# TritonDataCenter/containerpilot

Hardware: NVIDIA H100
Metric: events/sec through Bus.Publish (deliveries/s = 32-byte records landed in subscriber mailboxes) (higher is better)
Workload: dtype u8

## Files before the change

containerpilot_b200/csrc/cpbus.cu:

```cuda
#include "cpbus_kernels.cuh"

#include <algorithm>
#include <chrono>
#include <cstdio>
#include <cstdlib>
#include <cstring>
#include <deque>
#include <mutex>
#include <new>
#include <string>
#include <thread>
#include <unordered_map>
#include <vector>

using namespace cpbus_dev;

namespace {

thread_local char g_cuda_err[256] = "";

#define CK(call)                                                                                   \
  do {                                                                                             \
    cudaError_t e_ = (call);                                                                       \
    if (e_ != cudaSuccess) {                                                                       \
// ... 74 lines not shown
  unsigned long long* d_follow_clock = nullptr;
  int follow_next = 0;
  cudaEvent_t follow_done = nullptr;
  std::recursive_mutex follow_mu;
  DevPubAcct* d_acct = nullptr;
  DevPubAcct* h_acct = nullptr;
  std::deque<DbgItem> dbg_pending;
  PairCounter pub_pairs;
  cpbus_event* d_drain = nullptr; size_t drain_cap = 0;
  uint2* d_drain_idx = nullptr; size_t drain_idx_cap = 0;
  unsigned long long* d_ready_lb = nullptr; size_t ready_lb_tiles = 0;
  cpbus_ready* d_ready = nullptr; uint32_t* d_ready_slot = nullptr; size_t ready_stage_cap = 0;
  unsigned long long* h_ready_hdr = nullptr;
  unsigned long long* d_ready_hdr = nullptr;
  uint32_t subs_per_warp = 0;
  uint32_t order_block = 0;
  bool pdl = true;
  cudaEvent_t launched = nullptr;
  int hints = -1;
  static constexpr int kFoldSlots = 8;
  unsigned long long* d_fold = nullptr;
  cudaEvent_t fold_done[kFoldSlots] = {};
  uint32_t fold_next = 0;
  static constexpr int kStage = 8;
  static constexpr int kDevSlots = 64, kDevEpoch = 16;
  cpbus_event* d_stage = nullptr;
  cudaEvent_t epoch_done[kDevSlots / kDevEpoch] = {};
  uint32_t dev_slot = 0;
  cpbus_event* h_batch[kStage] = {};
  cudaEvent_t h2d_done[kStage] = {};
  cudaStream_t copy_stream = nullptr;
  cudaStream_t result_stream = nullptr;
  DevResultSlot* d_result = nullptr;
  DevResultSlot* h_result = nullptr;
  cudaEvent_t result_done[8] = {};
  uint32_t result_next = 0;
  DevStats* h_stats = nullptr;
  unsigned long long* h_fold = nullptr;
  int cur = 0;
  size_t n_staged = 0;

  std::vector<uint32_t> h_mask;
  std::vector<uint8_t> h_active;
  std::vector<uint8_t> h_npairs;
  uint2* d_pairs = nullptr;
  uint32_t n_paired = 0;
  uint32_t* d_order = nullptr;
  uint32_t n_order = 0, n_filtered = 0;
  bool order_dirty = true;
  std::vector<size_t> oneshot_idx;
  std::vector<HostTimer> h_timers;
  uint32_t n_next = 0, n_active = 0, n_timers = 0;
  uint64_t min_period = UINT64_MAX;

  uint64_t now = 0, last_watermark = 0, seq = 0;
  uint64_t room_lb = 0;

  int dbg_head = -1, dbg_tail = 0;
  cpbus_event dbg[10]{};

  std::unordered_map<std::string, uint32_t> intern;
  std::vector<std::string> sources;
  size_t intern_bytes = 0;
  struct EphSlot { std::string s; uint32_t gen = 0; bool live = false; };
  std::vector<EphSlot> eph;
  std::unordered_map<std::string, uint32_t> eph_map;
  uint32_t eph_next = 0;
  uint64_t eph_live = 0, eph_recycled = 0;
  std::vector<cpbus_stream*> streams;

  cpbus_stats_t st{};
  std::mutex mu;
};

namespace {

int rebuild_order(cpbus* b);

int dev_guard(cpbus* b) {
  CK(cudaSetDevice(b->device));
  return CPBUS_OK;
}

int stream_error(const cpbus* b) {
  const unsigned int e = *(volatile const unsigned int*)b->h_err;
  return (e & kErrFollowOrder) ? CPBUS_EORDER : (e ? CPBUS_ETIMEDOUT : CPBUS_OK);
}

uint32_t mask_word(const cpbus* b, uint32_t local) {
  uint32_t hint = 0;
  if (b->K && !b->h_timers.empty())
    for (uint32_t k = 0; k < b->K; k++)
// ... 38 lines not shown
    const size_t base = order.size();
    order.resize(base + count.back());
    for (uint32_t i = lo; i < hi; i++) if (!active || active[i]) order[base + count[masks[i] & CPBUS_MASK_ALL]++] = i;
    if (heavy_first) {
      const size_t nb = order.size() - base;
      uint32_t pc_count[34] = {};
      for (size_t k = 0; k < nb; k++) pc_count[32 - __builtin_popcount(masks[order[base + k]] & CPBUS_MASK_ALL) + 1]++;
      for (int k = 1; k < 34; k++) pc_count[k] += pc_count[k - 1];
      tmp.resize(nb);
      for (size_t k = 0; k < nb; k++) tmp[pc_count[32 - __builtin_popcount(masks[order[base + k]] & CPBUS_MASK_ALL)]++] = order[base + k];
      std::copy(tmp.begin(), tmp.end(), order.begin() + base);
    }
  }
}

int rebuild_order(cpbus* b) {
  std::vector<uint32_t> order;
  static_assert(sizeof(b->h_active[0]) == 1, "h_active is a byte vector");
  mask_order(b->h_mask.data(), reinterpret_cast<const uint8_t*>(b->h_active.data()), b->n_next, b->R, b->order_block, true, order);
  b->n_order = (uint32_t)order.size();
  if (b->n_order) {
    CK(cudaMemcpyAsync(b->d_order, order.data(), (size_t)b->n_order * 4, cudaMemcpyHostToDevice, b->stream));
    CK(cudaStreamSynchronize(b->stream));
  }
  b->order_dirty = false;
  return CPBUS_OK;
}

constexpr int kFanoutMaxSmem = 200 * 1024;

template <int STORE, bool TIMERS, bool DIGEST, bool ORDERED, bool PAIRS = false>
int launch_fanout_t(cpbus* b, const FanoutParams& p, uint32_t grid, size_t smem, bool follow) {
  static bool attr_done[2][64] = {};
  void (*kernel)(FanoutParams) = follow ? fanout_follow_kernel<STORE, TIMERS, DIGEST, ORDERED, PAIRS>
                                        : fanout_kernel<STORE, TIMERS, DIGEST, ORDERED, PAIRS>;
  const int dev = b->device & 63;
  if (!attr_done[follow][dev]) {
    CK(cudaFuncSetAttribute(kernel, cudaFuncAttributeMaxDynamicSharedMemorySize, kFanoutMaxSmem));
    attr_done[follow][dev] = true;
  }
  cudaLaunchConfig_t cfg{};
  cfg.gridDim = dim3(grid); cfg.blockDim = dim3(kThreads); cfg.dynamicSmemBytes = smem; cfg.stream = b->stream;
  cudaLaunchAttribute attr[1];
  attr[0].id = cudaLaunchAttributeProgrammaticStreamSerialization;
  attr[0].val.programmaticStreamSerializationAllowed = 1;
  cfg.attrs = attr; cfg.numAttrs = b->pdl ? 1 : 0;
  CK(cudaLaunchKernelEx(&cfg, kernel, p));
  CK(cudaGetLastError());
  return CPBUS_OK;
}
// ... 32 lines not shown
    p.follow_from_host = sa->follow_from_host ? 1u : 0u;
  }
  p.prefetch_src = prefetch_src; p.prefetch_dst = prefetch_dst; p.prefetch_n = prefetch_n;
  p.batch_dep = batch_dep ? 1u : 0u; p.n_ev = n;
  p.n_subs = b->n_next; p.ring_cap = b->R; p.K = b->K; p.sub_base = b->cfg.sub_id_base;
  p.use_digest = b->use_digest; p.lossless = b->lossless; p.timers_on = b->n_timers > 0 && b->K > 0;
  p.smem_cap = (n + 31u) & ~31u;
  const size_t hot_bytes = (size_t)b->n_next * (sizeof(SubCtl) + (p.timers_on ? b->K * sizeof(DevTimer) : 0));
  p.hints = b->hints >= 0 ? (uint32_t)b->hints : (hot_bytes <= (64u << 20) ? 1u : 0u);
  const uint32_t need = (b->n_next + kWarpsPerCta - 1) / kWarpsPerCta;
  uint32_t grid = b->cfg.grid_ctas ? std::max(1u, std::min(b->cfg.grid_ctas, need)) : 0u;
  int rc;
  const bool pairs_on = b->n_paired > 0 && b->d_pairs;
  p.pairs = pairs_on ? b->d_pairs : nullptr;
  size_t smem = fanout_smem_bytes(p.smem_cap) + (pairs_on ? kPairFilterBytes : 0);
  if (!pairs_on && !p.timers_on && b->n_filtered > 0) {
    if (b->order_dirty) { const int rc_order = rebuild_order(b); if (rc_order) return rc_order; }
    if (b->n_order) {
      const uint32_t scale = std::max(1u, (p.n_ev + 128u) / 256u);
      uint32_t spw = b->subs_per_warp ? std::min(32u, b->subs_per_warp)
                                      : std::max(4u, std::min(16u / scale, b->n_order / (20480u * scale)));
      p.order = b->d_order; p.n_order = b->n_order; p.spw = spw;
      const uint32_t warps = (b->n_order + spw - 1) / spw;
      grid = std::max(1u, (warps + kWarpsPerCta - 1) / kWarpsPerCta);
    }
  }
  if (pairs_on && !b->cfg.grid_ctas) {
    const uint32_t blocks = (b->n_next + 31u) / 32u;
    grid = std::max(1u, std::min((blocks + kWarpsPerCta - 1) / kWarpsPerCta, (uint32_t)b->sm_count * 16u));
  }
  if (!pairs_on && !p.order) {
    uint32_t spw = b->subs_per_warp;
    if (grid) spw = std::max(1u, (need + grid - 1) / grid);
    else if (!spw) {
      const uint32_t scale = std::max(1u, (p.n_ev + 128u) / 256u);
      const uint32_t cap = std::max(1u, 16u / scale);
      spw = std::max(1u, std::min(cap, (need + (uint32_t)b->sm_count * 7 * scale) / ((uint32_t)b->sm_count * 14 * scale)));
    }
    p.spw = spw;
    grid = std::max(1u, (need + spw - 1) / spw);
    const size_t off = fanout_stage_off(p.smem_cap);
    const size_t per_sub = sizeof(SubCtl) + (p.timers_on ? (size_t)b->K * sizeof(DevTimer) : 0);
    const size_t min_round = (size_t)kWarpsPerCta * per_sub;
    const size_t ctas = std::max<size_t>(1, std::min<size_t>(kCtasPerSm, b->smem_per_sm / (off + min_round + b->smem_reserved)));
    const size_t room = std::min<size_t>(kFanoutMaxSmem, b->smem_per_sm / ctas - b->smem_reserved) - off;
    p.stage_subs = std::max<uint32_t>(kWarpsPerCta, (uint32_t)std::min<size_t>((size_t)kWarpsPerCta * spw, room / per_sub) & ~7u);
    smem = off + p.stage_subs * per_sub;
  }
  const int variant = pairs_on ? (p.use_digest ? 7 : 6) : (p.timers_on ? 2 : 0) | (p.use_digest ? 1 : 0) | (p.order ? 4 : 0);
#define CPBUS_DISPATCH(ST)                                                                \
  switch (variant) {                                                                     \
    case 0: rc = launch_fanout_t<ST, false, false, false>(b, p, grid, smem, follow); break;      \
    case 1: rc = launch_fanout_t<ST, false, true, false>(b, p, grid, smem, follow); break;       \
    case 2: rc = launch_fanout_t<ST, true, false, false>(b, p, grid, smem, follow); break;       \
    case 3: rc = launch_fanout_t<ST, true, true, false>(b, p, grid, smem, follow); break;        \
    case 4: rc = launch_fanout_t<ST, false, false, true>(b, p, grid, smem, follow); break;       \
    case 5: rc = launch_fanout_t<ST, false, true, true>(b, p, grid, smem, follow); break;        \
    case 6: rc = launch_fanout_t<ST, true, false, false, true>(b, p, grid, smem, follow); break; \
    default: rc = launch_fanout_t<ST, true, true, false, true>(b, p, grid, smem, follow); break; \
  }
  switch (b->store) {
    case CPBUS_STORE_V4: CPBUS_DISPATCH(CPBUS_STORE_V4); break;
    case CPBUS_STORE_BULK: CPBUS_DISPATCH(CPBUS_STORE_BULK); break;
    default: CPBUS_DISPATCH(CPBUS_STORE_V8); break;
// ... 206 lines not shown
  int ndev = 0;
  if (cudaGetDeviceCount(&ndev) != cudaSuccess || ndev == 0) {
    snprintf(g_cuda_err, sizeof(g_cuda_err), "no CUDA device visible");
    return CPBUS_ENODEV;
  }
  cpbus* b = new (std::nothrow) cpbus();
  if (!b) return CPBUS_ENOMEM;
  b->cfg = *cfg; b->cfg.ring_cap = R; b->cfg.batch_cap = B;
  b->N = cfg->n_max_subs; b->R = R; b->B = B; b->K = K;
  b->lossless = cfg->flags & CPBUS_CFG_LOSSLESS; b->use_digest = cfg->flags & CPBUS_CFG_DIGEST;
  b->room_lb = R;
  b->store = cfg->store_path == CPBUS_STORE_AUTO ? CPBUS_STORE_V8 : (int)cfg->store_path;
  if (const char* e = getenv("CPBUS_PDL")) b->pdl = atoi(e) != 0;
  if (const char* e = getenv("CPBUS_HINTS")) b->hints = atoi(e);
  if (const char* e = getenv("CPBUS_SUBS_PER_WARP")) b->subs_per_warp = (uint32_t)atoi(e);
  if (const char* e = getenv("CPBUS_ORDER_BLOCK")) b->order_block = (uint32_t)atoll(e);
  int rc = CPBUS_OK;
  auto fail = [&](int code) { cpbus_destroy(b); return code; };
  if (cfg->device >= 0) b->device = cfg->device;
  else if (cudaGetDevice(&b->device) != cudaSuccess) return fail(CPBUS_ECUDA);
  if (b->device >= ndev) return fail(CPBUS_EINVAL);
  if ((rc = dev_guard(b))) return fail(rc);
  cudaDeviceProp prop{};
  if (cudaGetDeviceProperties(&prop, b->device) == cudaSuccess) {
    b->sm_count = prop.multiProcessorCount;
    b->smem_per_sm = prop.sharedMemPerMultiprocessor; b->smem_reserved = prop.reservedSharedMemPerBlock;
  }
  if (cfg->stream) b->stream = (cudaStream_t)cfg->stream;
  else {
    if (cudaStreamCreateWithFlags(&b->stream, cudaStreamNonBlocking) != cudaSuccess) return fail(CPBUS_ECUDA);
    b->own_stream = true;
  }
  const size_t N = b->N;
#define ALLOC(ptr, bytes)                                                                     \
  if (cudaMalloc((void**)&(ptr), (bytes)) != cudaSuccess) {                                   \
    snprintf(g_cuda_err, sizeof(g_cuda_err), "cudaMalloc(%zu) failed", (size_t)(bytes));     \
    return fail(CPBUS_ENOMEM);                                                                \
  }
  ALLOC(b->d_ring, N * R * sizeof(cpbus_event));
  ALLOC(b->d_ctl, N * sizeof(SubCtl)); ALLOC(b->d_order, N * 4);
  if (K) ALLOC(b->d_timers, N * K * sizeof(DevTimer));
  ALLOC(b->d_stats, sizeof(DevStats)); ALLOC(b->d_fold, 32 * cpbus::kFoldSlots); ALLOC(b->d_pow, kPowTableLen * 8);
  ALLOC(b->d_desc, 2 * ((fanout_desc_bytes(2048) + 255) & ~(size_t)255)); ALLOC(b->d_desc_ready, 256);
  if (cudaMemsetAsync(b->d_desc_ready, 0, 256, b->stream) != cudaSuccess) return fail(CPBUS_ECUDA);
  if (cudaStreamCreateWithFlags(&b->copy_stream, cudaStreamNonBlocking) != cudaSuccess) return fail(CPBUS_ECUDA);
  if (cudaStreamCreateWithFlags(&b->result_stream, cudaStreamNonBlocking) != cudaSuccess) return fail(CPBUS_ECUDA);
  if (cudaEventCreateWithFlags(&b->launched, cudaEventDisableTiming) != cudaSuccess) return fail(CPBUS_ECUDA);
  ALLOC(b->d_stage, (size_t)cpbus::kDevSlots * B * sizeof(cpbus_event));
  for (int i = 0; i < cpbus::kDevSlots / cpbus::kDevEpoch; i++)
    if (cudaEventCreateWithFlags(&b->epoch_done[i], cudaEventDisableTiming) != cudaSuccess) return fail(CPBUS_ECUDA);
  for (int i = 0; i < cpbus::kStage; i++) {
    if (cudaMallocHost((void**)&b->h_batch[i], (size_t)B * sizeof(cpbus_event)) != cudaSuccess) return fail(CPBUS_ENOMEM);
    if (cudaEventCreateWithFlags(&b->h2d_done[i], cudaEventDisableTiming) != cudaSuccess) return fail(CPBUS_ECUDA);
  }
  ALLOC(b->d_batch_local, (size_t)B * sizeof(cpbus_event));
// ... 34 lines not shown
  b->intern.emplace(std::string(), 0u);
  b->sources.emplace_back();
  *out = b;
  return CPBUS_OK;
} CPBUS_CATCH

int cpbus_destroy(cpbus_t* b) try {
  if (!b) return CPBUS_EINVAL;
  follow_resolve(b);
  cudaSetDevice(b->device);
  if (b->stream) cudaStreamSynchronize(b->stream);
  while (!b->streams.empty()) cpbus_stream_close(b->streams.back());
  if (b->h_follow) cudaFreeHost(b->h_follow);
  cudaFree(b->d_follow_clock);
  if (b->follow_done) cudaEventDestroy(b->follow_done);
  cudaFree(b->d_ring); cudaFree(b->d_ctl); cudaFree(b->d_order); cudaFree(b->d_pairs);
  cudaFree(b->d_timers); cudaFree(b->d_stats); cudaFree(b->d_fold); cudaFree(b->d_pow); cudaFree(b->d_desc); cudaFree(b->d_desc_ready);
  if (b->copy_stream) cudaStreamSynchronize(b->copy_stream);
  if (b->result_stream) { cudaStreamSynchronize(b->result_stream); cudaStreamDestroy(b->result_stream); }
  for (int i = 0; i < cpbus::kStage; i++) {
    if (b->h_batch[i]) cudaFreeHost(b->h_batch[i]);
    if (b->h2d_done[i]) cudaEventDestroy(b->h2d_done[i]);
  }
  cudaFree(b->d_stage);
  for (int i = 0; i < cpbus::kDevSlots / cpbus::kDevEpoch; i++) if (b->epoch_done[i]) cudaEventDestroy(b->epoch_done[i]);
  if (b->copy_stream) cudaStreamDestroy(b->copy_stream);
  if (b->launched) cudaEventDestroy(b->launched);
  cudaFree(b->d_drain); cudaFree(b->d_drain_idx);
  cudaFree(b->d_ready_lb); cudaFree(b->d_ready); cudaFree(b->d_ready_slot);
  if (b->h_ready_hdr) cudaFreeHost(b->h_ready_hdr);
  cudaFree(b->d_result); cudaFree(b->d_batch_local); cudaFree(b->d_admit_batch); cudaFree(b->d_pf_buf); cudaFree(b->d_pf_state); cudaFree(b->d_acct);
// ... 71 lines not shown
  if ((uint64_t)b->n_next + n > b->N) return CPBUS_ENOSPC;
  int rc = dev_guard(b); if (rc) return rc;
  if ((rc = follow_resolve(b))) return rc;
  if ((rc = flush_staged(b, b->now))) return rc;
  const uint32_t first = b->n_next;
  std::vector<SubCtl> blocks(n);
  memset(blocks.data(), 0, (size_t)n * sizeof(SubCtl));
  for (uint32_t i = 0; i < n; i++) {
    b->h_mask[first + i] = (masks ? masks[i] : CPBUS_MASK_ALL) & CPBUS_MASK_ALL;
    blocks[i].mask = b->h_mask[first + i] | kActiveBit;
    b->h_active[first + i] = 1;
    if (b->h_mask[first + i] != CPBUS_MASK_ALL) b->n_filtered++;
  }
  CK(cudaMemcpyAsync(b->d_ctl + first, blocks.data(), (size_t)n * sizeof(SubCtl), cudaMemcpyHostToDevice, b->stream));
  CK(cudaStreamSynchronize(b->stream));
  b->n_next += n; b->n_active += n; b->order_dirty = true;
  if (first_sub_id) *first_sub_id = b->cfg.sub_id_base + first;
  return CPBUS_OK;
} CPBUS_CATCH

int cpbus_subscribe(cpbus_t* b, uint32_t mask, uint32_t* sub_id) { return cpbus_subscribe_many(b, &mask, 1, sub_id); }

static int push_mask_words(cpbus* b, uint32_t first, uint32_t n);

int cpbus_subscribe_pairs(cpbus_t* b, uint32_t mask, const cpbus_pair* pairs, uint32_t n_pairs, uint32_t* sub_id) try {
  if (!b || n_pairs > CPBUS_MAX_PAIRS || (n_pairs && !pairs)) return CPBUS_EINVAL;
  for (uint32_t j = 0; j < n_pairs; j++) if (pairs[j].code >= CPBUS_N_CODES) return CPBUS_EINVAL;
  uint2 row[CPBUS_MAX_PAIRS];
  uint32_t used = 0;
  for (uint32_t j = 0; j < n_pairs; j++)
    if (!((mask >> pairs[j].code) & 1u)) row[used++] = make_uint2(pairs[j].code, pairs[j].source_id);
// ... 60 lines not shown
  if (first_sub_id) *first_sub_id = first;
  return CPBUS_OK;
} CPBUS_CATCH

int cpbus_unsubscribe(cpbus_t* b, uint32_t sub_id) try {
  if (!b) return CPBUS_EINVAL;
  const uint32_t l = sub_id - b->cfg.sub_id_base;
  if (sub_id < b->cfg.sub_id_base || l >= b->n_next) return CPBUS_ENOENT;
  int rc = dev_guard(b); if (rc) return rc;
  if ((rc = follow_resolve(b))) return rc;
  if ((rc = flush_staged(b, b->now))) return rc;
  if (!b->h_active[l]) return CPBUS_ECLOSED;
  b->h_active[l] = 0;
  if (b->h_mask[l] != CPBUS_MASK_ALL) b->n_filtered--;
  if (!b->h_npairs.empty() && b->h_npairs[l]) { b->h_npairs[l] = 0; b->n_paired--; }
  b->order_dirty = true;
  const uint32_t word = 0;
  CK(cudaMemcpyAsync(&b->d_ctl[l].mask, &word, 4, cudaMemcpyHostToDevice, b->stream));
  if (b->K && !b->h_timers.empty()) {
    for (uint32_t k = 0; k < b->K; k++) {
      HostTimer& t = b->h_timers[(size_t)l * b->K + k];
      if (t.active) { t.active = false; b->n_timers--; }
    }
    CK(cudaMemsetAsync(b->d_timers + (size_t)l * b->K, 0xFF, b->K * sizeof(DevTimer), b->stream));
  }
  CK(cudaStreamSynchronize(b->stream));
  b->n_active--;
  return CPBUS_OK;
} CPBUS_CATCH

int cpbus_set_mask(cpbus_t* b, uint32_t sub_id, uint32_t mask) try {
  if (!b) return CPBUS_EINVAL;
  const uint32_t l = sub_id - b->cfg.sub_id_base;
  if (sub_id < b->cfg.sub_id_base || l >= b->n_next) return CPBUS_ENOENT;
  if (!b->h_active[l]) return CPBUS_ECLOSED;
  int rc = dev_guard(b); if (rc) return rc;
  if ((rc = follow_resolve(b))) return rc;
  if ((rc = flush_staged(b, b->now))) return rc;
  mask &= CPBUS_MASK_ALL;
  if (b->h_mask[l] != CPBUS_MASK_ALL) b->n_filtered--;
  if (mask != CPBUS_MASK_ALL) b->n_filtered++;
  b->h_mask[l] = mask; b->order_dirty = true;
  return push_mask_words(b, l, 1);
} CPBUS_CATCH

static int push_mask_words(cpbus* b, uint32_t first, uint32_t n) {
  std::vector<uint32_t> words(n);
  for (uint32_t i = 0; i < n; i++) words[i] = mask_word(b, first + i);
  CK(cudaMemcpy2DAsync(&b->d_ctl[first].mask, sizeof(SubCtl), words.data(), 4, 4, n, cudaMemcpyHostToDevice, b->stream));
  CK(cudaStreamSynchronize(b->stream));
  return CPBUS_OK;
}

int cpbus_timer_add(cpbus_t* b, uint32_t sub_id, uint64_t period_ns, uint32_t source_id, int oneshot, uint32_t* timer_id) try {
  if (!b || !period_ns) return CPBUS_EINVAL;
  if (!b->K) return CPBUS_ENOSPC;
  const uint32_t l = sub_id - b->cfg.sub_id_base;
// ... 1026 lines not shown
```

containerpilot_b200/csrc/cpbus_fanout_body.cuh:

```cuda
  constexpr bool STAGED = !ORDERED && !PAIRS;
  extern __shared__ __align__(128) unsigned char smem[];
  const uint32_t cap = p.smem_cap;
  cpbus_event* s_batch = reinterpret_cast<cpbus_event*>(smem);
  uint64_t* s_rhash = reinterpret_cast<uint64_t*>(smem + (size_t)cap * 32);
  uint2* s_meta = reinterpret_cast<uint2*>(smem + (size_t)cap * 40);
  uint64_t* s_q = reinterpret_cast<uint64_t*>(smem + (size_t)cap * 48);
  uint32_t* s_dsum = reinterpret_cast<uint32_t*>(s_q + cap + 2);
  uint32_t* s_present = s_dsum + 40;
  uint64_t* s_pow = s_q + cap + 2 + 20 + (PAIRS ? kPairFilterWords / 2 : 0);
  BatchSummary* s_sum = reinterpret_cast<BatchSummary*>(s_pow + cap + 66);
  uint32_t* s_tick = reinterpret_cast<uint32_t*>(s_sum + 1);
  const uint4* s_ctl4 = reinterpret_cast<const uint4*>(smem + fanout_stage_off(cap));
  const uint4* s_tim4 = s_ctl4 + 2u * p.stage_subs;

  const int tid = threadIdx.x, lane = tid & 31, warp = tid >> 5;
  uint32_t n = FOLLOW ? 0u : p.n_ev;
  uint64_t w_follow = 0;

  if (p.batch_dep) asm volatile("griddepcontrol.wait;" ::: "memory");
  const bool stream = p.staged == 2u;
  const uint32_t pf_slot = stream ? (uint32_t)(p.stream_seq % kStreamPrefetch) : 0u;
  uint32_t pos = ORDERED ? (blockIdx.x * kWarpsPerCta + warp) * p.spw : 0u;
  uint32_t my_ids = 0;
  if (ORDERED && pos + lane < min(pos + p.spw, p.n_order)) my_ids = __ldg(p.order + pos + lane);
  if (tid == 0) {
    mbar_init(&s_sum->mbar, 1); mbar_init(&s_sum->mbar_desc, 1); mbar_init(&s_sum->mbar_state, 1);
    s_sum->acc_deliv = 0; s_sum->acc_ticks = 0; s_sum->acc_dig_lo = 0; s_sum->acc_dig_hi = 0;
    s_sum->stream_local = (stream && !p.lossless && p.stream_off == 0 && __ldcg(p.pf_state + pf_slot) == p.stream_seq) ? 1u : 0u;
    s_sum->own_desc = blockIdx.x == 0 ? 1u : 0u; s_sum->abort_launch = 0;
  }
  __syncthreads();
  const bool stream_local = stream && s_sum->stream_local;
  const bool staged = FOLLOW || (p.staged && !stream_local);
  const cpbus_event* batch_src = stream_local ? p.pf_buf + (size_t)pf_slot * p.pf_stride : p.batch;
  if (tid == 0) {
    const uint32_t pow_bytes = ((cap + 65u) * 8u + 15u) & ~15u;
    const bool direct = n && !staged;
    mbar_expect_tx(&s_sum->mbar, (direct ? n * 32u : 0u) + pow_bytes);
    if (direct) bulk_g2s(s_batch, batch_src, n * 32u, &s_sum->mbar);
// ... 190 lines not shown
      __threadfence();
      __syncthreads();
      if (tid == 0) {
        const unsigned long long flag = p.launch_seq | (ab ? kAbortBit : 0ull);
        asm volatile("st.release.gpu.global.u64 [%0], %1;" ::"l"(p.desc_ready), "l"(flag) : "memory");
      }
    }
  } else {
    mbar_wait(&s_sum->mbar_desc, 0);
    if constexpr (FOLLOW) {
      n = s_sum->abort_launch ? 0u : s_dsum[kFollowN];
      w_follow = ((uint64_t)s_dsum[kFollowWHi] << 32) | s_dsum[kFollowWLo];
    }
    mbar_wait(&s_sum->mbar, (staged && n && !s_sum->abort_launch) ? 1u : 0u);
  }
  constexpr bool PLANAR = STORE != CPBUS_STORE_BULK && !ORDERED;
  const uint32_t hi_off = cap;
  if (PLANAR && n) {
    uint4* sq = reinterpret_cast<uint4*>(s_batch);
    uint4 v[8];
    __syncthreads();
#pragma unroll
    for (int r = 0; r < 8; r++) { const uint32_t q = tid + r * kThreads; if (q < 2u * n) v[r] = sq[q]; }
    __syncthreads();
#pragma unroll
    for (int r = 0; r < 8; r++) { const uint32_t q = tid + r * kThreads; if (q < 2u * n) sq[(q & 1u) * hi_off + (q >> 1)] = v[r]; }
    __syncthreads();
  }
  auto ev_ts = [&](uint32_t i) -> uint64_t {
    return PLANAR ? reinterpret_cast<const uint64_t*>(reinterpret_cast<const uint4*>(s_batch) + i)[1] : s_batch[i].ts_ns;
  };
  auto ev_code_src = [&](uint32_t i) -> uint2 {
    return PLANAR ? reinterpret_cast<const uint2*>(reinterpret_cast<const uint4*>(s_batch) + hi_off + i)[0] : make_uint2(s_batch[i].code, s_batch[i].source_id);
  };
  const bool aborted = s_sum->abort_launch != 0;
  const uint32_t K = p.K, J = K ? 32u / K : 32u;
  const uint32_t tk_slot = lane / J, tk_j = lane % J;
  const bool timers_on = TIMERS && p.timers_on && K;
  const uint32_t wstride = gridDim.x * kWarpsPerCta;
  uint32_t pos_end = (aborted || !ORDERED) ? 0u : min(pos + p.spw, p.n_order);
  const uint32_t pos_step = ORDERED ? 1u : kWarpsPerCta;
  const uint32_t pos0 = pos;
  uint32_t s = ORDERED ? __shfl_sync(0xffffffffu, my_ids, 0) : pos;
  if (!p.batch_dep) asm volatile("griddepcontrol.wait;" ::: "memory");
  asm volatile("griddepcontrol.launch_dependents;");
  const uint32_t rng_first = blockIdx.x * kWarpsPerCta * p.spw, rng_end = min(rng_first + kWarpsPerCta * p.spw, p.n_subs);
  auto stage_round = [&](uint32_t first) {
    if (!STAGED || tid != 0 || aborted || first >= rng_end) return;
    const uint32_t rn = min(p.stage_subs, rng_end - first);
    asm volatile("fence.proxy.async.shared::cta;" ::: "memory");
    const uint32_t tim_bytes = timers_on ? rn * K * (uint32_t)sizeof(DevTimer) : 0u;
    mbar_expect_tx(&s_sum->mbar_state, rn * (uint32_t)sizeof(SubCtl) + tim_bytes);
    bulk_g2s_hint(const_cast<uint4*>(s_ctl4), p.ctl + first, rn * (uint32_t)sizeof(SubCtl), &s_sum->mbar_state, keep);
    if (tim_bytes) bulk_g2s_hint(const_cast<uint4*>(s_tim4), p.timers + (size_t)first * K, tim_bytes, &s_sum->mbar_state, keep);
  };
  uint4 ca = make_uint4(0, 0, 0, 0), cb = ca, ta = ca;
  if (ORDERED && pos < pos_end) ld_sector(p.ctl + s, ca, cb, keep);
  const uint32_t present = s_dsum[0];
  const bool has_unicast = s_dsum[1] != 0;
  bool bulk_pending = false;
  uint32_t tri_blk = blockIdx.x * kWarpsPerCta + warp, tri_base = 0, tri_live = 0;
  uint4 tri_a = make_uint4(0, 0, 0, 0), tri_b = tri_a;
  uint32_t rnd_first = rng_first, rnd_phase = 0;
  for (;;) {
  if constexpr (STAGED) {
    if (aborted || rnd_first >= rng_end) break;
    stage_round(rnd_first);
    mbar_wait(&s_sum->mbar_state, rnd_phase);
    rnd_phase ^= 1u;
    pos = rnd_first + warp; pos_end = rnd_first + min(p.stage_subs, rng_end - rnd_first);
  }
  if constexpr (PAIRS) {
    bool exhausted = aborted;
    while (!tri_live && !exhausted) {
      tri_base = tri_blk * 32u;
      if (tri_base >= p.n_subs) { exhausted = true; break; }
      tri_blk += wstride;
      const uint32_t sl = tri_base + lane;
      bool live = false;
      tri_a = make_uint4(0, 0, 0, 0); tri_b = tri_a;
      if (sl < p.n_subs) ld_sector(p.ctl + sl, tri_a, tri_b, keep);
      const uint32_t ml = tri_b.z;
      if (ml & kActiveBit) {
        live = has_unicast || (ml & present) != 0;
        if (!live && timers_on) {
// ... 24 lines not shown
    const uint32_t jl = (uint32_t)__ffs(tri_live) - 1u;
    tri_live &= tri_live - 1u;
    pos = tri_base + jl; pos_end = pos + 1u; s = pos;
    ca = make_uint4(__shfl_sync(0xffffffffu, tri_a.x, jl), __shfl_sync(0xffffffffu, tri_a.y, jl), __shfl_sync(0xffffffffu, tri_a.z, jl), __shfl_sync(0xffffffffu, tri_a.w, jl));
    cb = make_uint4(__shfl_sync(0xffffffffu, tri_b.x, jl), __shfl_sync(0xffffffffu, tri_b.y, jl), __shfl_sync(0xffffffffu, tri_b.z, jl), __shfl_sync(0xffffffffu, tri_b.w, jl));
    if (timers_on && tk_slot < K) ld_half(p.timers + (size_t)s * K + tk_slot, ta, keep);
  }
  const uint32_t Rm = p.ring_cap - 1;
  const uint4* s4 = reinterpret_cast<const uint4*>(s_batch);
  const uint32_t scratch_words = max(32u, cap / 2u);
  uint32_t* my_tick = s_tick + warp * scratch_words;

  uint32_t run_mask = 0xffffffffu, run_k = 0;
  uint64_t run_sum = 0;
  for (; pos < pos_end; pos += pos_step) {
    const uint32_t si = pos - rnd_first;
    uint4 cur_a = ca, cur_b = cb;
    auto ctl_half = [&](uint32_t h) -> uint4 { return STAGED ? s_ctl4[2u * si + h] : (h ? cur_b : cur_a); };
    auto tim_half = [&](uint32_t h) -> uint4 {
      if (STAGED) return s_tim4[2u * (si * K + tk_slot) + h];
      if (!h) return ta;
      uint4 cold;
      ld_half(reinterpret_cast<const unsigned char*>(p.timers + (size_t)s * K + tk_slot) + 16, cold, keep);
      return cold;
    };
    if (STAGED) { cur_a = ctl_half(0); cur_b = ctl_half(1); }
    if (ORDERED) s = __shfl_sync(0xffffffffu, my_ids, (pos - pos0) & 31); else s = pos;
    if (ORDERED) {
      const uint32_t pn = pos + pos_step;
      if (pn < pos_end) ld_sector(p.ctl + __shfl_sync(0xffffffffu, my_ids, (pn - pos0) & 31), ca, cb, keep);
    }
    const uint32_t m = cur_b.z;
    if (!(m & kActiveBit)) continue;
    const uint64_t tail = ((uint64_t)cur_a.y << 32) | cur_a.x;
    cpbus_event* ring = p.ring + (size_t)s * p.ring_cap;
    const uint32_t gid = p.sub_base + s;
    const uint32_t nslots = timers_on ? min((m >> kTimerHintShift) & 0xFu, K) : 0u;
    const bool dense = !has_unicast && ((m & present) == present);

    uint32_t n_ticks = 0, tk_mask = 0, tk_rank = 0, tk_src = 0, tk_fired = 0;
    bool tk_valid = false; uint64_t tk_due = 0, tk_period = 0;
    if (nslots) {
      uint64_t tk_due0 = kTimerIdle;
      if (TIMERS && tk_slot < nslots) {
        const uint4 hot = tim_half(0);
        tk_due0 = ((uint64_t)hot.y << 32) | hot.x; tk_period = ((uint64_t)hot.w << 32) | hot.z;
// ... 110 lines not shown
        const uint64_t w3 = (uint64_t)gid | ((uint64_t)CPBUS_F_TICK << 32);
        const uint4 a = make_uint4((uint32_t)w0, (uint32_t)(w0 >> 32), (uint32_t)w1, (uint32_t)(w1 >> 32));
        const uint4 b = make_uint4((uint32_t)w2, (uint32_t)(w2 >> 32), (uint32_t)w3, (uint32_t)(w3 >> 32));
        st_v8(ring + (((uint32_t)tail + out) & Rm), a, b);
        if (DIGEST) {
          const uint32_t prev = tk_rank ? my_tick[tk_rank - 1] : 0u;
          dsum = (s_q[tk_pos] - s_q[prev]) * s_pow[n_ticks - tk_rank] + record_hash_words(w0, w1, w2, w3) * s_pow[k - 1 - out];
          if (tk_rank == n_ticks - 1) dsum += s_q[n] - s_q[tk_pos];
        }
      }
      if (DIGEST) dsum = warp_sum64(dsum);
      __syncwarp();
    } else if (!(PAIRS && pair_live) && !has_unicast && n_ticks == 0) {
      if constexpr (!TIMERS) {
        uint16_t* my_idx = reinterpret_cast<uint16_t*>(my_tick);
        const bool reuse = ORDERED && (m & CPBUS_MASK_ALL) == run_mask;
        if (!reuse) {
          uint32_t base = 0;
          const uint32_t nchunks = (n + 31) >> 5;
          for (uint32_t c0 = 0; c0 < nchunks; c0 += 4) {
            uint32_t cbit[4];
#pragma unroll
            for (uint32_t u = 0; u < 4; u++) {
              const uint32_t i = (c0 + u) * 32 + lane;
              cbit[u] = i < n ? s_meta[i].x : 0u;
            }
#pragma unroll
            for (uint32_t u = 0; u < 4; u++) {
              const bool match = (m & cbit[u]) != 0;
              const uint32_t w = __ballot_sync(0xffffffffu, match);
              if (match) my_idx[base + __popc(w & ((1u << lane) - 1u))] = (uint16_t)((c0 + u) * 32 + lane);
// ... 14 lines not shown
          const uint32_t n0 = o + 64 < k ? my_idx[o + 64] : 0u, n1 = o + 96 < k ? my_idx[o + 96] : 0u;
          copy_record_pairs<PLANAR>(s4, hi_off, ring, (uint32_t)tail, Rm, i0, o, v0);
          copy_record_pairs<PLANAR>(s4, hi_off, ring, (uint32_t)tail, Rm, i1, o + 32, v1);
          if (hashing) {
            if (v0) acc = acc * p32 + s_rhash[i0];
            if (v1) acc = acc * p32 + s_rhash[i1];
          }
          i0 = n0; i1 = n1;
        }
        if (DIGEST) {
          if (reuse) dsum = run_sum;
          else {
            const uint32_t cnt = k > (uint32_t)lane ? (k - lane + 31u) / 32u : 0u;
            dsum = cnt ? acc * s_pow[k - 1 - (lane + 32u * (cnt - 1u))] : 0ull;
            dsum = warp_sum64(dsum);
            if (ORDERED) run_sum = dsum;
          }
        }
        if (ORDERED) run_mask = m & CPBUS_MASK_ALL;
        __syncwarp();
      } else {
        uint32_t kk = ((m >> lane) & 1u) ? s_dsum[2 + lane] : 0u;
        kk = __reduce_add_sync(0xffffffffu, kk);
        k = kk;
        uint32_t base = 0;
        const uint32_t nchunks = (n + 31) >> 5;
        for (uint32_t c = 0; c < nchunks; c++) {
          const uint32_t i = c * 32 + lane;
          const bool match = i < n && (m & s_meta[i].x) != 0;
          const uint32_t w = __ballot_sync(0xffffffffu, match);
          const uint32_t out = base + __popc(w & ((1u << lane) - 1u));
          if (DIGEST && match) dsum += s_rhash[i] * s_pow[k - 1 - out];
          copy_record_pairs<PLANAR>(s4, hi_off, ring, (uint32_t)tail, Rm, i, out, match);
          base += __popc(w);
// ... 98 lines not shown
      const uint64_t dig = ((uint64_t)c1.y << 32) | c1.x;
      const uint64_t nt = tail + k;
      const uint64_t nd = DIGEST ? dig * s_pow[k] + dsum : dig;
      st_sector(p.ctl + s, make_uint4((uint32_t)nt, (uint32_t)(nt >> 32), c0.z, c0.w),
                make_uint4((uint32_t)nd, (uint32_t)(nd >> 32), m, 0u), keep);
      atomicAdd(&s_sum->acc_deliv, k);
      if (DIGEST) {
        const uint32_t f = (uint32_t)nd ^ (uint32_t)(nd >> 32);
        atomicAdd(&s_sum->acc_dig_lo, f & 0xFFFFu);
        atomicAdd(&s_sum->acc_dig_hi, f >> 16);
      }
      if (TIMERS && n_ticks) atomicAdd(&s_sum->acc_ticks, n_ticks);
    }
  }

  if constexpr (ORDERED) break;
  if constexpr (STAGED) {
    __syncthreads();
    rnd_first += p.stage_subs;
  }
  }
  if (STORE == CPBUS_STORE_BULK && bulk_pending && lane == 0)
    asm volatile("cp.async.bulk.wait_group 0;" ::: "memory");
  __syncthreads();
  if (tid == 0) {
    DevStatSlot* st = &p.stats->slot[blockIdx.x % kStatSlots];
    if (s_sum->acc_deliv) atomicAdd(&st->deliveries, (unsigned long long)s_sum->acc_deliv);
    if (s_sum->acc_ticks) atomicAdd(&st->ticks, (unsigned long long)s_sum->acc_ticks);
    DevResultSlot* rs = &p.result[blockIdx.x % kResultSub];
    if (s_sum->acc_deliv) atomicAdd(&rs->deliveries, (unsigned long long)s_sum->acc_deliv);
    if (s_sum->acc_ticks) atomicAdd(&rs->ticks, (unsigned long long)s_sum->acc_ticks);
// ... 72 lines not shown
```

containerpilot_b200/csrc/cpbus_kernels.cuh:

```cuda
#pragma once
#include <cstdint>
#include <cuda_runtime.h>

#include "../../include/cpbus.h"

namespace cpbus_dev {

constexpr int kWarpsPerCta = 8;
constexpr int kThreads = kWarpsPerCta * 32;
constexpr int kCtasPerSm = 4;
constexpr uint32_t kActiveBit = 0x80000000u;
constexpr int kTimerHintShift = 24;
constexpr uint32_t kPairBit = 0x10000000u;
constexpr uint32_t kPairNone = 0xFFFFFFFFu;
constexpr uint32_t kPairFilterWords = 1024;
constexpr uint32_t kPairFilterBytes = kPairFilterWords * 4;
__host__ __device__ inline uint32_t pair_key_hash(uint32_t code, uint32_t source_id) {
  uint32_t x = (source_id ^ (code << 27)) * 0x9E3779B1u;
  x ^= x >> 15; x *= 0x85EBCA77u; x ^= x >> 13;
  return x;
}
constexpr uint64_t kDigestP = 0x9E3779B97F4A7C15ull;
constexpr uint32_t kPowTableLen = 2048 + 65 + 7;

// ... 73 lines not shown
  SubCtl* ctl;
  DevTimer* timers;
  DevStats* stats;
  const uint64_t* pow_table;
  unsigned char* desc;
  unsigned long long* desc_ready;
  unsigned long long launch_seq;
  DevResultSlot* result;
  DevResultSlot* result_next;
  cpbus_event* batch_local;
  uint32_t staged;
  const cpbus_event* prefetch_src;
  cpbus_event* prefetch_dst;
  uint32_t prefetch_n;
  uint32_t batch_dep;
  const uint32_t* order;
  uint32_t n_order, spw;
  uint32_t stage_subs;
  uint64_t w_now;
  uint32_t n_ev, n_subs, ring_cap, K, sub_base;
  uint32_t use_digest, lossless, timers_on;
  uint32_t smem_cap;
  uint32_t hints;
  const uint2* pairs;
  const StreamHdr* stream_hdr;
  unsigned long long* stream_ack;
  unsigned long long stream_seq;
  const StreamHdr* stream_next_hdr;
  uint32_t stream_off;
  uint32_t stream_final;
  unsigned long long* pf_state;
  cpbus_event* pf_buf;
// ... 133 lines not shown
  uint32_t stream_local;
  uint32_t own_desc;
  uint32_t abort_launch;
  uint32_t pf_ok;
  uint64_t red[kWarpsPerCta];
};

__host__ __device__ inline size_t fanout_desc_bytes(uint32_t cap) { return (size_t)24 * cap + 16 + 160 + kPairFilterBytes; }

__host__ __device__ inline size_t fanout_smem_bytes(uint32_t cap) {
  const size_t scratch = (cap / 2u > 32u ? cap / 2u : 32u) * sizeof(uint32_t);
  return (size_t)cap * 56 + 16 + 160 + (size_t)(cap + 66) * 8 + sizeof(BatchSummary) + kWarpsPerCta * scratch + 128;
}
__host__ __device__ inline size_t fanout_stage_off(uint32_t cap) { return (fanout_smem_bytes(cap) + 127) & ~(size_t)127; }

template <int STORE, bool TIMERS, bool DIGEST, bool ORDERED, bool PAIRS = false>
__global__ void __launch_bounds__(kThreads, kCtasPerSm) fanout_kernel(const FanoutParams p) {
  constexpr bool FOLLOW = false;
#include "cpbus_fanout_body.cuh"
}
template <int STORE, bool TIMERS, bool DIGEST, bool ORDERED, bool PAIRS = false>
__global__ void __launch_bounds__(kThreads, kCtasPerSm) fanout_follow_kernel(const FanoutParams p) {
  constexpr bool FOLLOW = true;
#include "cpbus_fanout_body.cuh"
}

__global__ void admit_kernel(const cpbus_event* batch, uint32_t n_ev, uint64_t w_now, const SubCtl* ctl,
                             const DevTimer* timers, uint32_t n_subs, uint32_t ring_cap, uint32_t K, uint32_t sub_base,
                             uint32_t timers_on, DevStats* stats, const uint2* pairs) {
  __shared__ uint32_t hist[32];
  __shared__ uint32_t s_uni;
  __shared__ unsigned long long s_max;
  if (threadIdx.x < 32) hist[threadIdx.x] = 0;
  if (threadIdx.x == 0) { s_uni = 0; s_max = 0; }
  __syncthreads();
  for (uint32_t i = threadIdx.x; i < n_ev; i += blockDim.x) {
// ... 309 lines not shown
```

Baseline: 93.14 billion.

## Replace host-built global subscriber order with per-round in-smem mask sort

Removes the host-side mask ordering (rebuild_order with a synchronous H2D upload) and the ORDERED kernel path that gathered subscriber control blocks through an index array. Instead, the staged path now sorts each shared-memory round of subscribers by popcount and mask using an O(n^2) rank sort, so runs of identical masks can reuse computed digests while the staged bulk loads are kept. It also caps CTAs per SM at 2 when the grid exceeds the resident capacity and hands the full remaining shared memory to each block. The quadratic per-round sort and the added __syncthreads cost extra work, and the sort only groups masks within a round, not globally.

```diff
diff --git a/containerpilot_b200/csrc/cpbus.cu b/containerpilot_b200/csrc/cpbus.cu
--- a/containerpilot_b200/csrc/cpbus.cu
+++ b/containerpilot_b200/csrc/cpbus.cu
@@ -112,7 +112,6 @@
   unsigned long long* h_ready_hdr = nullptr;
   unsigned long long* d_ready_hdr = nullptr;
   uint32_t subs_per_warp = 0;
-  uint32_t order_block = 0;
   bool pdl = true;
   cudaEvent_t launched = nullptr;
   int hints = -1;
@@ -143,9 +142,7 @@
   std::vector<uint8_t> h_npairs;
   uint2* d_pairs = nullptr;
   uint32_t n_paired = 0;
-  uint32_t* d_order = nullptr;
-  uint32_t n_order = 0, n_filtered = 0;
-  bool order_dirty = true;
+  uint32_t n_filtered = 0;
   std::vector<size_t> oneshot_idx;
   std::vector<HostTimer> h_timers;
   uint32_t n_next = 0, n_active = 0, n_timers = 0;
@@ -172,8 +169,6 @@
 };
 
 namespace {
-
-int rebuild_order(cpbus* b);
 
 int dev_guard(cpbus* b) {
   CK(cudaSetDevice(b->device));
@@ -242,26 +237,14 @@
   }
 }
 
-int rebuild_order(cpbus* b) {
-  std::vector<uint32_t> order;
-  static_assert(sizeof(b->h_active[0]) == 1, "h_active is a byte vector");
-  mask_order(b->h_mask.data(), reinterpret_cast<const uint8_t*>(b->h_active.data()), b->n_next, b->R, b->order_block, true, order);
-  b->n_order = (uint32_t)order.size();
-  if (b->n_order) {
-    CK(cudaMemcpyAsync(b->d_order, order.data(), (size_t)b->n_order * 4, cudaMemcpyHostToDevice, b->stream));
-    CK(cudaStreamSynchronize(b->stream));
-  }
-  b->order_dirty = false;
-  return CPBUS_OK;
-}
-
 constexpr int kFanoutMaxSmem = 200 * 1024;
-
-template <int STORE, bool TIMERS, bool DIGEST, bool ORDERED, bool PAIRS = false>
+constexpr int kRingCtasPerSm = 2;
+
+template <int STORE, bool TIMERS, bool DIGEST, bool SORTED, bool PAIRS = false>
 int launch_fanout_t(cpbus* b, const FanoutParams& p, uint32_t grid, size_t smem, bool follow) {
   static bool attr_done[2][64] = {};
-  void (*kernel)(FanoutParams) = follow ? fanout_follow_kernel<STORE, TIMERS, DIGEST, ORDERED, PAIRS>
-                                        : fanout_kernel<STORE, TIMERS, DIGEST, ORDERED, PAIRS>;
+  void (*kernel)(FanoutParams) = follow ? fanout_follow_kernel<STORE, TIMERS, DIGEST, SORTED, PAIRS>
+                                        : fanout_kernel<STORE, TIMERS, DIGEST, SORTED, PAIRS>;
   const int dev = b->device & 63;
   if (!attr_done[follow][dev]) {
     CK(cudaFuncSetAttribute(kernel, cudaFuncAttributeMaxDynamicSharedMemorySize, kFanoutMaxSmem));
@@ -324,22 +307,12 @@
   const bool pairs_on = b->n_paired > 0 && b->d_pairs;
   p.pairs = pairs_on ? b->d_pairs : nullptr;
   size_t smem = fanout_smem_bytes(p.smem_cap) + (pairs_on ? kPairFilterBytes : 0);
-  if (!pairs_on && !p.timers_on && b->n_filtered > 0) {
-    if (b->order_dirty) { const int rc_order = rebuild_order(b); if (rc_order) return rc_order; }
-    if (b->n_order) {
-      const uint32_t scale = std::max(1u, (p.n_ev + 128u) / 256u);
-      uint32_t spw = b->subs_per_warp ? std::min(32u, b->subs_per_warp)
-                                      : std::max(4u, std::min(16u / scale, b->n_order / (20480u * scale)));
-      p.order = b->d_order; p.n_order = b->n_order; p.spw = spw;
-      const uint32_t warps = (b->n_order + spw - 1) / spw;
-      grid = std::max(1u, (warps + kWarpsPerCta - 1) / kWarpsPerCta);
-    }
-  }
+  const bool sorted = !pairs_on && !p.timers_on && b->n_filtered > 0;
   if (pairs_on && !b->cfg.grid_ctas) {
     const uint32_t blocks = (b->n_next + 31u) / 32u;
     grid = std::max(1u, std::min((blocks + kWarpsPerCta - 1) / kWarpsPerCta, (uint32_t)b->sm_count * 16u));
   }
-  if (!pairs_on && !p.order) {
+  if (!pairs_on) {
     uint32_t spw = b->subs_per_warp;
     if (grid) spw = std::max(1u, (need + grid - 1) / grid);
     else if (!spw) {
@@ -350,14 +323,15 @@
     p.spw = spw;
     grid = std::max(1u, (need + spw - 1) / spw);
     const size_t off = fanout_stage_off(p.smem_cap);
-    const size_t per_sub = sizeof(SubCtl) + (p.timers_on ? (size_t)b->K * sizeof(DevTimer) : 0);
+    const size_t per_sub = sizeof(SubCtl) + (p.timers_on ? (size_t)b->K * sizeof(DevTimer) : 0) + (sorted ? 8 : 0);
     const size_t min_round = (size_t)kWarpsPerCta * per_sub;
-    const size_t ctas = std::max<size_t>(1, std::min<size_t>(kCtasPerSm, b->smem_per_sm / (off + min_round + b->smem_reserved)));
+    const size_t max_ctas = grid > (uint32_t)(kCtasPerSm * b->sm_count) ? kRingCtasPerSm : kCtasPerSm;
+    const size_t ctas = std::max<size_t>(1, std::min<size_t>(max_ctas, b->smem_per_sm / (off + min_round + b->smem_reserved)));
     const size_t room = std::min<size_t>(kFanoutMaxSmem, b->smem_per_sm / ctas - b->smem_reserved) - off;
     p.stage_subs = std::max<uint32_t>(kWarpsPerCta, (uint32_t)std::min<size_t>((size_t)kWarpsPerCta * spw, room / per_sub) & ~7u);
-    smem = off + p.stage_subs * per_sub;
-  }
-  const int variant = pairs_on ? (p.use_digest ? 7 : 6) : (p.timers_on ? 2 : 0) | (p.use_digest ? 1 : 0) | (p.order ? 4 : 0);
+    smem = off + room;
+  }
+  const int variant = pairs_on ? (p.use_digest ? 7 : 6) : (p.timers_on ? 2 : 0) | (p.use_digest ? 1 : 0) | (sorted ? 4 : 0);
 #define CPBUS_DISPATCH(ST)                                                                \
   switch (variant) {                                                                     \
     case 0: rc = launch_fanout_t<ST, false, false, false>(b, p, grid, smem, follow); break;      \
@@ -594,7 +568,6 @@
   if (const char* e = getenv("CPBUS_PDL")) b->pdl = atoi(e) != 0;
   if (const char* e = getenv("CPBUS_HINTS")) b->hints = atoi(e);
   if (const char* e = getenv("CPBUS_SUBS_PER_WARP")) b->subs_per_warp = (uint32_t)atoi(e);
-  if (const char* e = getenv("CPBUS_ORDER_BLOCK")) b->order_block = (uint32_t)atoll(e);
   int rc = CPBUS_OK;
   auto fail = [&](int code) { cpbus_destroy(b); return code; };
   if (cfg->device >= 0) b->device = cfg->device;
@@ -618,7 +591,7 @@
     return fail(CPBUS_ENOMEM);                                                                \
   }
   ALLOC(b->d_ring, N * R * sizeof(cpbus_event));
-  ALLOC(b->d_ctl, N * sizeof(SubCtl)); ALLOC(b->d_order, N * 4);
+  ALLOC(b->d_ctl, N * sizeof(SubCtl));
   if (K) ALLOC(b->d_timers, N * K * sizeof(DevTimer));
   ALLOC(b->d_stats, sizeof(DevStats)); ALLOC(b->d_fold, 32 * cpbus::kFoldSlots); ALLOC(b->d_pow, kPowTableLen * 8);
   ALLOC(b->d_desc, 2 * ((fanout_desc_bytes(2048) + 255) & ~(size_t)255)); ALLOC(b->d_desc_ready, 256);
@@ -683,7 +656,7 @@
   if (b->h_follow) cudaFreeHost(b->h_follow);
   cudaFree(b->d_follow_clock);
   if (b->follow_done) cudaEventDestroy(b->follow_done);
-  cudaFree(b->d_ring); cudaFree(b->d_ctl); cudaFree(b->d_order); cudaFree(b->d_pairs);
+  cudaFree(b->d_ring); cudaFree(b->d_ctl); cudaFree(b->d_pairs);
   cudaFree(b->d_timers); cudaFree(b->d_stats); cudaFree(b->d_fold); cudaFree(b->d_pow); cudaFree(b->d_desc); cudaFree(b->d_desc_ready);
   if (b->copy_stream) cudaStreamSynchronize(b->copy_stream);
   if (b->result_stream) { cudaStreamSynchronize(b->result_stream); cudaStreamDestroy(b->result_stream); }
@@ -785,7 +758,7 @@
   }
   CK(cudaMemcpyAsync(b->d_ctl + first, blocks.data(), (size_t)n * sizeof(SubCtl), cudaMemcpyHostToDevice, b->stream));
   CK(cudaStreamSynchronize(b->stream));
-  b->n_next += n; b->n_active += n; b->order_dirty = true;
+  b->n_next += n; b->n_active += n;
   if (first_sub_id) *first_sub_id = b->cfg.sub_id_base + first;
   return CPBUS_OK;
 } CPBUS_CATCH
@@ -876,7 +849,6 @@
   b->h_active[l] = 0;
   if (b->h_mask[l] != CPBUS_MASK_ALL) b->n_filtered--;
   if (!b->h_npairs.empty() && b->h_npairs[l]) { b->h_npairs[l] = 0; b->n_paired--; }
-  b->order_dirty = true;
   const uint32_t word = 0;
   CK(cudaMemcpyAsync(&b->d_ctl[l].mask, &word, 4, cudaMemcpyHostToDevice, b->stream));
   if (b->K && !b->h_timers.empty()) {
@@ -902,7 +874,7 @@
   mask &= CPBUS_MASK_ALL;
   if (b->h_mask[l] != CPBUS_MASK_ALL) b->n_filtered--;
   if (mask != CPBUS_MASK_ALL) b->n_filtered++;
-  b->h_mask[l] = mask; b->order_dirty = true;
+  b->h_mask[l] = mask;
   return push_mask_words(b, l, 1);
 } CPBUS_CATCH
 
diff --git a/containerpilot_b200/csrc/cpbus_fanout_body.cuh b/containerpilot_b200/csrc/cpbus_fanout_body.cuh
--- a/containerpilot_b200/csrc/cpbus_fanout_body.cuh
+++ b/containerpilot_b200/csrc/cpbus_fanout_body.cuh
@@ -1,4 +1,4 @@
-  constexpr bool STAGED = !ORDERED && !PAIRS;
+  constexpr bool STAGED = !PAIRS;
   extern __shared__ __align__(128) unsigned char smem[];
   const uint32_t cap = p.smem_cap;
   cpbus_event* s_batch = reinterpret_cast<cpbus_event*>(smem);
@@ -12,6 +12,8 @@
   uint32_t* s_tick = reinterpret_cast<uint32_t*>(s_sum + 1);
   const uint4* s_ctl4 = reinterpret_cast<const uint4*>(smem + fanout_stage_off(cap));
   const uint4* s_tim4 = s_ctl4 + 2u * p.stage_subs;
+  uint32_t* s_key = const_cast<uint32_t*>(reinterpret_cast<const uint32_t*>(s_tim4));
+  uint32_t* s_rank = s_key + p.stage_subs;
 
   const int tid = threadIdx.x, lane = tid & 31, warp = tid >> 5;
   uint32_t n = FOLLOW ? 0u : p.n_ev;
@@ -20,9 +22,7 @@
   if (p.batch_dep) asm volatile("griddepcontrol.wait;" ::: "memory");
   const bool stream = p.staged == 2u;
   const uint32_t pf_slot = stream ? (uint32_t)(p.stream_seq % kStreamPrefetch) : 0u;
-  uint32_t pos = ORDERED ? (blockIdx.x * kWarpsPerCta + warp) * p.spw : 0u;
-  uint32_t my_ids = 0;
-  if (ORDERED && pos + lane < min(pos + p.spw, p.n_order)) my_ids = __ldg(p.order + pos + lane);
+  uint32_t pos = 0;
   if (tid == 0) {
     mbar_init(&s_sum->mbar, 1); mbar_init(&s_sum->mbar_desc, 1); mbar_init(&s_sum->mbar_state, 1);
     s_sum->acc_deliv = 0; s_sum->acc_ticks = 0; s_sum->acc_dig_lo = 0; s_sum->acc_dig_hi = 0;
@@ -243,7 +243,7 @@
     }
     mbar_wait(&s_sum->mbar, (staged && n && !s_sum->abort_launch) ? 1u : 0u);
   }
-  constexpr bool PLANAR = STORE != CPBUS_STORE_BULK && !ORDERED;
+  constexpr bool PLANAR = STORE != CPBUS_STORE_BULK;
   const uint32_t hi_off = cap;
   if (PLANAR && n) {
     uint4* sq = reinterpret_cast<uint4*>(s_batch);
@@ -267,10 +267,9 @@
   const uint32_t tk_slot = lane / J, tk_j = lane % J;
   const bool timers_on = TIMERS && p.timers_on && K;
   const uint32_t wstride = gridDim.x * kWarpsPerCta;
-  uint32_t pos_end = (aborted || !ORDERED) ? 0u : min(pos + p.spw, p.n_order);
-  const uint32_t pos_step = ORDERED ? 1u : kWarpsPerCta;
-  const uint32_t pos0 = pos;
-  uint32_t s = ORDERED ? __shfl_sync(0xffffffffu, my_ids, 0) : pos;
+  uint32_t pos_end = 0;
+  const uint32_t pos_step = SORTED ? 1u : kWarpsPerCta;
+  uint32_t s = pos;
   if (!p.batch_dep) asm volatile("griddepcontrol.wait;" ::: "memory");
   asm volatile("griddepcontrol.launch_dependents;");
   const uint32_t rng_first = blockIdx.x * kWarpsPerCta * p.spw, rng_end = min(rng_first + kWarpsPerCta * p.spw, p.n_subs);
@@ -284,7 +283,6 @@
     if (tim_bytes) bulk_g2s_hint(const_cast<uint4*>(s_tim4), p.timers + (size_t)first * K, tim_bytes, &s_sum->mbar_state, keep);
   };
   uint4 ca = make_uint4(0, 0, 0, 0), cb = ca, ta = ca;
-  if (ORDERED && pos < pos_end) ld_sector(p.ctl + s, ca, cb, keep);
   const uint32_t present = s_dsum[0];
   const bool has_unicast = s_dsum[1] != 0;
   bool bulk_pending = false;
@@ -297,7 +295,25 @@
     stage_round(rnd_first);
     mbar_wait(&s_sum->mbar_state, rnd_phase);
     rnd_phase ^= 1u;
-    pos = rnd_first + warp; pos_end = rnd_first + min(p.stage_subs, rng_end - rnd_first);
+    if constexpr (SORTED) {
+      const uint32_t rn = min(p.stage_subs, rng_end - rnd_first);
+      for (uint32_t i = tid; i < rn; i += kThreads) {
+        const uint32_t mi = s_ctl4[2u * i + 1u].z, mc = mi & CPBUS_MASK_ALL;
+        s_key[i] = (mi & kActiveBit) ? ((uint32_t)(32 - __popc(mc)) << 17) | mc : 0xFFFFFFFFu;
+      }
+      __syncthreads();
+      for (uint32_t i = tid; i < rn; i += kThreads) {
+        const uint32_t ki = s_key[i];
+        uint32_t r = 0;
+        for (uint32_t j = 0; j < rn; j++) { const uint32_t kj = s_key[j]; r += (kj < ki || (kj == ki && j < i)) ? 1u : 0u; }
+        s_rank[r] = i;
+      }
+      __syncthreads();
+      const uint32_t per = (rn + kWarpsPerCta - 1) / kWarpsPerCta;
+      pos = min(rn, warp * per); pos_end = min(rn, pos + per);
+    } else {
+      pos = rnd_first + warp; pos_end = rnd_first + min(p.stage_subs, rng_end - rnd_first);
+    }
   }
   if constexpr (PAIRS) {
     bool exhausted = aborted;
@@ -352,7 +368,7 @@
   uint32_t run_mask = 0xffffffffu, run_k = 0;
   uint64_t run_sum = 0;
   for (; pos < pos_end; pos += pos_step) {
-    const uint32_t si = pos - rnd_first;
+    const uint32_t si = SORTED ? s_rank[pos] : pos - rnd_first;
     uint4 cur_a = ca, cur_b = cb;
     auto ctl_half = [&](uint32_t h) -> uint4 { return STAGED ? s_ctl4[2u * si + h] : (h ? cur_b : cur_a); };
     auto tim_half = [&](uint32_t h) -> uint4 {
@@ -363,11 +379,7 @@
       return cold;
     };
     if (STAGED) { cur_a = ctl_half(0); cur_b = ctl_half(1); }
-    if (ORDERED) s = __shfl_sync(0xffffffffu, my_ids, (pos - pos0) & 31); else s = pos;
-    if (ORDERED) {
-      const uint32_t pn = pos + pos_step;
-      if (pn < pos_end) ld_sector(p.ctl + __shfl_sync(0xffffffffu, my_ids, (pn - pos0) & 31), ca, cb, keep);
-    }
+    s = SORTED ? rnd_first + si : pos;
     const uint32_t m = cur_b.z;
     if (!(m & kActiveBit)) continue;
     const uint64_t tail = ((uint64_t)cur_a.y << 32) | cur_a.x;
@@ -508,7 +520,7 @@
     } else if (!(PAIRS && pair_live) && !has_unicast && n_ticks == 0) {
       if constexpr (!TIMERS) {
         uint16_t* my_idx = reinterpret_cast<uint16_t*>(my_tick);
-        const bool reuse = ORDERED && (m & CPBUS_MASK_ALL) == run_mask;
+        const bool reuse = SORTED && (m & CPBUS_MASK_ALL) == run_mask;
         if (!reuse) {
           uint32_t base = 0;
           const uint32_t nchunks = (n + 31) >> 5;
@@ -553,10 +565,10 @@
             const uint32_t cnt = k > (uint32_t)lane ? (k - lane + 31u) / 32u : 0u;
             dsum = cnt ? acc * s_pow[k - 1 - (lane + 32u * (cnt - 1u))] : 0ull;
             dsum = warp_sum64(dsum);
-            if (ORDERED) run_sum = dsum;
-          }
-        }
-        if (ORDERED) run_mask = m & CPBUS_MASK_ALL;
+            if (SORTED) run_sum = dsum;
+          }
+        }
+        if (SORTED) run_mask = m & CPBUS_MASK_ALL;
         __syncwarp();
       } else {
         uint32_t kk = ((m >> lane) & 1u) ? s_dsum[2 + lane] : 0u;
@@ -685,7 +697,6 @@
     }
   }
 
-  if constexpr (ORDERED) break;
   if constexpr (STAGED) {
     __syncthreads();
     rnd_first += p.stage_subs;
diff --git a/containerpilot_b200/csrc/cpbus_kernels.cuh b/containerpilot_b200/csrc/cpbus_kernels.cuh
--- a/containerpilot_b200/csrc/cpbus_kernels.cuh
+++ b/containerpilot_b200/csrc/cpbus_kernels.cuh
@@ -111,8 +111,7 @@
   cpbus_event* prefetch_dst;
   uint32_t prefetch_n;
   uint32_t batch_dep;
-  const uint32_t* order;
-  uint32_t n_order, spw;
+  uint32_t spw;
   uint32_t stage_subs;
   uint64_t w_now;
   uint32_t n_ev, n_subs, ring_cap, K, sub_base;
@@ -276,12 +275,12 @@
 }
 __host__ __device__ inline size_t fanout_stage_off(uint32_t cap) { return (fanout_smem_bytes(cap) + 127) & ~(size_t)127; }
 
-template <int STORE, bool TIMERS, bool DIGEST, bool ORDERED, bool PAIRS = false>
+template <int STORE, bool TIMERS, bool DIGEST, bool SORTED, bool PAIRS = false>
 __global__ void __launch_bounds__(kThreads, kCtasPerSm) fanout_kernel(const FanoutParams p) {
   constexpr bool FOLLOW = false;
 #include "cpbus_fanout_body.cuh"
 }
-template <int STORE, bool TIMERS, bool DIGEST, bool ORDERED, bool PAIRS = false>
+template <int STORE, bool TIMERS, bool DIGEST, bool SORTED, bool PAIRS = false>
 __global__ void __launch_bounds__(kThreads, kCtasPerSm) fanout_follow_kernel(const FanoutParams p) {
   constexpr bool FOLLOW = true;
 #include "cpbus_fanout_body.cuh"
```

Result: faster. 94.74 billion (median of 6 runs) (+1.7%).
